# huangjh-pub/di-fusion

Hardware: AMD Instinct MI355X
Metric: frames/s integrate+decode+mesh, 640x480 synthetic stream (higher is better)
Workload: dtype f32

## Files before the change

### di_fusion_amd/csrc/common.hip.h

```cpp
#pragma once
#include <hip/hip_runtime.h>
#include <stdint.h>

#include "../../include/difusion.h"

#define DIF_WAVE 64
#define DIF_BLOCK 256
#define DIF_INVALID_KEY 0xFFFFFFFFu
#define NO_PACKED_F32 _Pragma("clang loop vectorize(disable) interleave(disable)")

#define DIF_CHECK_LAUNCH()                                   \
    do {                                                     \
        if (hipGetLastError() != hipSuccess) return DIF_ELAUNCH; \
    } while (0)

namespace dif {

struct Geo {
    int nx, ny, nz;
    float bx, by, bz, vs;
};

__host__ inline Geo geo_of(const dif_map_t* m) {
    Geo g;
    g.nx = m->nx; g.ny = m->ny; g.nz = m->nz;
    g.bx = m->bound_min[0]; g.by = m->bound_min[1]; g.bz = m->bound_min[2];
    g.vs = m->voxel_size;
    return g;
}

__device__ __forceinline__ int xcd_run_item(int b, int n, int max_run) {
    if (b >= n) return b;
    for (int base = 0, rem = n; rem >= 16;) {
        int R = 1 << (28 - __clz(rem));
        if (R > max_run) R = max_run;
        if (b < base + 8 * R) { const int l = b - base; return base + (l & 7) * R + (l >> 3); }
        base += 8 * R; rem -= 8 * R;
    }
    return b;
}

__device__ __forceinline__ int lane_id() { return (int)(threadIdx.x & 63); }

__device__ __forceinline__ float normalize1(float p, float b, float vs) { return __fdiv_rn(__fsub_rn(p, b), vs); }

__device__ __forceinline__ bool voxel_of(const Geo& g, float x, float y, float z, float& xnx, float& xny, float& xnz,
                                         int& ix, int& iy, int& iz) {
    xnx = normalize1(x, g.bx, g.vs);
    xny = normalize1(y, g.by, g.vs);
    xnz = normalize1(z, g.bz, g.vs);
    float cx = ceilf(xnx), cy = ceilf(xny), cz = ceilf(xnz);
    bool ok = (cx >= 1.0f) && (cy >= 1.0f) && (cz >= 1.0f) && (cx <= (float)g.nx) && (cy <= (float)g.ny) && (cz <= (float)g.nz);
    ix = ok ? (int)cx - 1 : 0;
    iy = ok ? (int)cy - 1 : 0;
    iz = ok ? (int)cz - 1 : 0;
    return ok;
}

__device__ __forceinline__ int linearize(const Geo& g, int ix, int iy, int iz) { return iz + g.nz * iy + (g.nz * g.ny) * ix; }

__device__ __forceinline__ void unlinearize(const Geo& g, int lin, int& ix, int& iy, int& iz) {
    ix = lin / (g.ny * g.nz);
    iy = (lin / g.nz) % g.ny;
    iz = lin % g.nz;
}

__device__ __forceinline__ int clampi(int v, int lo, int hi) { return v < lo ? lo : (v > hi ? hi : v); }

struct GridMarks {
    uint32_t* bits; int* tot; int per_words;
    __device__ __forceinline__ void set(int v) const {
        const uint32_t b = 1u << (v & 31);
        const int w = v >> 5;
        const uint32_t old = atomicOr(bits + w, b);
        if (!(old & b)) atomicAdd(tot + w / per_words, 1);
    }
};

struct HaloLists {
    int32_t* list; int cap; int* counters;
    int64_t l_lo, l_hi, r_lo, r_hi;
    __device__ __forceinline__ void note(int slot, int64_t lin) const {
        if (!list) return;
        if (lin >= l_lo && lin < l_hi) { const int k = atomicAdd(counters + DIF_C_HALO_L, 1); if (k < cap) list[k] = slot; }
        if (lin >= r_lo && lin < r_hi) { const int k = atomicAdd(counters + DIF_C_HALO_R, 1); if (k < cap) list[cap + k] = slot; }
    }
};

__host__ inline bool map_is_tiled(const dif_map_t* m) { return m->own_x_hi > m->own_x_lo && (m->own_x_lo > 0 || m->own_x_hi < m->nx); }

__host__ inline HaloLists halo_lists_of(const dif_map_t* m) {
    HaloLists h = {};
    if (!m->halo_list || m->halo_list_cap <= 0 || !map_is_tiled(m) || m->halo <= 0) return h;
    const int64_t plane = (int64_t)m->ny * m->nz;
    h.list = m->halo_list; h.cap = m->halo_list_cap; h.counters = m->counters;
    if (m->own_x_lo > 0) { h.l_lo = m->own_x_lo * plane; h.l_hi = (int64_t)(m->own_x_lo + m->halo < m->own_x_hi ? m->own_x_lo + m->halo : m->own_x_hi) * plane; }
    if (m->own_x_hi < m->nx) { h.r_hi = m->own_x_hi * plane; h.r_lo = (int64_t)(m->own_x_hi - m->halo > m->own_x_lo ? m->own_x_hi - m->halo : m->own_x_lo) * plane; }
    return h;
}

template <int CTRL, int ROW_MASK>
__device__ __forceinline__ long long dpp_mov64(long long v) {
    const int lo = __builtin_amdgcn_update_dpp(0, (int)v, CTRL, ROW_MASK, 0xF, false);
    const int hi = __builtin_amdgcn_update_dpp(0, (int)(v >> 32), CTRL, ROW_MASK, 0xF, false);
    return ((long long)hi << 32) | (unsigned int)lo;
}

__device__ __forceinline__ long long seg_incl_scan32(long long v, int col, int my_head) {
    const int head_r = max(my_head, col & 16);
    long long u;
    u = dpp_mov64<0x111, 0xF>(v); if (col - 1 >= head_r) v += u;
    u = dpp_mov64<0x112, 0xF>(v); if (col - 2 >= head_r) v += u;
    u = dpp_mov64<0x114, 0xF>(v); if (col - 4 >= head_r) v += u;
    u = dpp_mov64<0x118, 0xF>(v); if (col - 8 >= head_r) v += u;
    u = dpp_mov64<0x142, 0xA>(v); if (col >= 16 && my_head < 16) v += u;
    return v;
}

__device__ __forceinline__ int wave_incl_scan(int v) {
    int lane = lane_id();
#pragma unroll
    for (int d = 1; d < 64; d <<= 1) {
        int o = __shfl_up(v, d);
        if (lane >= d) v += o;
    }
    return v;
}

__device__ __forceinline__ int block_excl_scan(int v, int* smem, int& total) {
    int lane = lane_id(), wid = threadIdx.x >> 6, nw = blockDim.x >> 6;
    int inc = wave_incl_scan(v);
    __syncthreads();
    if (lane == 63) smem[wid] = inc;
    __syncthreads();
    int base = 0, tot = 0;
    for (int w = 0; w < nw; ++w) {
        int s = smem[w];
        if (w < wid) base += s;
        tot += s;
    }
    total = tot;
    return base + inc - v;
}

__device__ __forceinline__ int block_sum(int v, int* smem) {
    int lane = lane_id(), wid = threadIdx.x >> 6, nw = blockDim.x >> 6;
#pragma unroll
    for (int d = 32; d >= 1; d >>= 1) v += __shfl_xor(v, d);
    __syncthreads();
    if (lane == 0) smem[wid] = v;
    __syncthreads();
    int tot = 0;
    for (int w = 0; w < nw; ++w) tot += smem[w];
    return tot;
}

__device__ __forceinline__ void scan_range(int n, int& lo, int& hi) {
    int per = (n + (int)gridDim.x - 1) / (int)gridDim.x;
    per = (per + DIF_BLOCK - 1) / DIF_BLOCK * DIF_BLOCK;
    long long l = (long long)blockIdx.x * per;
    lo = l < n ? (int)l : n;
    long long h = l + per;
    hi = h < n ? (int)h : n;
}

template <class F>
__global__ void __launch_bounds__(DIF_BLOCK) k_scan_pass1(F f, const int* n_ptr, int n_static, int* block_tot) {
    __shared__ int smem[8];
    int n = n_ptr ? *n_ptr : n_static;
    int lo, hi;
    scan_range(n, lo, hi);
    int c = 0;
    for (int i = lo + (int)threadIdx.x; i < hi; i += DIF_BLOCK) c += f.count(i);
    int tot = block_sum(c, smem);
    if (threadIdx.x == 0) block_tot[blockIdx.x] = tot;
}

template <class F>
__global__ void __launch_bounds__(DIF_BLOCK) k_scan_pass2(F f, const int* n_ptr, int n_static, const int* block_tot) {
    __shared__ int smem[8];
    int n = n_ptr ? *n_ptr : n_static;
    int lo, hi;
    scan_range(n, lo, hi);
    int before = 0, all = 0;
    for (int b = (int)threadIdx.x; b < (int)gridDim.x; b += DIF_BLOCK) {
        int t = block_tot[b];
        all += t;
        if (b < (int)blockIdx.x) before += t;
    }
    int offset = block_sum(before, smem);
    int total = block_sum(all, smem);
    for (int base = lo; base < hi; base += DIF_BLOCK) {
        int i = base + (int)threadIdx.x;
        int c = (i < hi) ? f.count(i) : 0;
        int chunk_total;
        int ex = block_excl_scan(c, smem, chunk_total);
        if (i < hi && c > 0) f.emit(i, offset + ex);
        offset += chunk_total;
    }
    if (blockIdx.x == 0 && threadIdx.x == 0) f.finish(total);
}

template <class F>
__global__ void __launch_bounds__(1024) k_scan_single(F f, const int* n_ptr, int n_static) {
    __shared__ int smem[16];
    const int n = n_ptr ? *n_ptr : n_static;
    const int per = (n + 1023) / 1024;
    const int lo = min(n, (int)threadIdx.x * per), hi = min(n, lo + per);
    int c = 0;
    for (int i = lo; i < hi; ++i) c += f.count(i);
    int total;
    int offset = block_excl_scan(c, smem, total);
    for (int i = lo; i < hi; ++i) {
        int ci = f.count(i);
        if (ci > 0) f.emit(i, offset);
        offset += ci;
    }
    if (threadIdx.x == 0) f.finish(total);
}

template <class A, int NS>
struct BatchN { A s[NS]; };
template <class A>
using Batch = BatchN<A, DIF_MAX_STREAMS>;

template <int NS, class T>
struct Ranges {
    T pre[NS + 1], cnt[NS];
    __device__ __forceinline__ T total() const { return pre[NS]; }
    __device__ __forceinline__ void locate(T x, int& sm, T& lt, T& n) const {
        sm = 0; lt = x; n = cnt[0];
#pragma unroll
        for (int j = 1; j < NS; ++j)
            if (x >= pre[j]) { sm = j; lt = x - pre[j]; n = cnt[j]; }
    }
};

template <class F>
struct ScanBatch { F f[DIF_MAX_STREAMS]; const int* tot[DIF_MAX_STREAMS]; };

template <class F>
__global__ void __launch_bounds__(DIF_BLOCK) k_scan_pass2_batch(ScanBatch<F> b, int n_static) {
    __shared__ int smem[8];
    const F& f = b.f[blockIdx.y];
    const int* __restrict__ block_tot = b.tot[blockIdx.y];
    const int n = n_static;
    int lo, hi;
    scan_range(n, lo, hi);
    int before = 0, all = 0;
    for (int k = (int)threadIdx.x; k < (int)gridDim.x; k += DIF_BLOCK) {
        int t = block_tot[k];
        all += t;
        if (k < (int)blockIdx.x) before += t;
    }
    int offset = block_sum(before, smem);
    int total = block_sum(all, smem);
    for (int base = lo; base < hi; base += DIF_BLOCK) {
        int i = base + (int)threadIdx.x;
        int c = (i < hi) ? f.count(i) : 0;
        int chunk_total;
        int ex = block_excl_scan(c, smem, chunk_total);
        if (i < hi && c > 0) f.emit(i, offset + ex);
        offset += chunk_total;
    }
    if (blockIdx.x == 0 && threadIdx.x == 0) f.finish(total);
}

template <class F>
__global__ void __launch_bounds__(1024) k_scan_single_batch(ScanBatch<F> b, int n_static) {
    __shared__ int smem[16];
// ... 106 lines not shown
```

### di_fusion_amd/csrc/kernels_integrate.hip.h

```cpp
#pragma once

__device__ __forceinline__ void voxel_count_point(const Geo& g, bool in_range, float x, float y, float z, int64_t i, int* __restrict__ pt_lin,
                                                  int* __restrict__ frame_count, int* __restrict__ counters, int px_lo, int px_hi) {
    const int lane = lane_id();
    if (i < 4) counters[DIF_C_ALLOC_NEW + i] = 0;
    int lin = -2;
    if (in_range) {
        float xn, yn, zn; int ix, iy, iz;
        bool ok = voxel_of(g, x, y, z, xn, yn, zn, ix, iy, iz);
        ok = ok && ix >= px_lo && ix < px_hi;
        lin = ok ? linearize(g, ix, iy, iz) : -1;
        pt_lin[i] = lin;
    }
    int prev = __shfl_up(lin, 1);
    bool head = (lane == 0) || (prev != lin);
    unsigned long long heads = __ballot(head);
    if (head && lin >= 0) {
        unsigned long long above = (lane == 63) ? 0ull : (heads >> (lane + 1));
        int run = above ? __ffsll((long long)above) : (64 - lane);
        atomicAdd(frame_count + lin, run);
    }
}

__global__ void __launch_bounds__(DIF_BLOCK) k_voxel_count(Geo g, const float* __restrict__ xyz, int64_t N, int* __restrict__ pt_lin,
                                                         int* __restrict__ frame_count, int* __restrict__ counters, int px_lo, int px_hi) {
    const int64_t i = (int64_t)blockIdx.x * blockDim.x + threadIdx.x;
    const bool in = i < N;
    voxel_count_point(g, in, in ? xyz[i * 3 + 0] : 0.f, in ? xyz[i * 3 + 1] : 0.f, in ? xyz[i * 3 + 2] : 0.f, i, pt_lin, frame_count, counters, px_lo, px_hi);
}

struct ImageGeo { int H, W; float fx, fy, cx, cy; };

struct PointSrc {
    const float* xyz; const float* normal;
    const dif_frame_t* frame; ImageGeo im;
};

__device__ __forceinline__ Pose pose_of(const dif_frame_t* __restrict__ frame) {
    Pose P;
#pragma unroll
    for (int k = 0; k < 9; ++k) P.r[k] = frame->pose[k];
#pragma unroll
    for (int k = 0; k < 3; ++k) P.t[k] = frame->pose[9 + k];
    return P;
}

__device__ __forceinline__ void src_point(const PointSrc& s, const Pose& P, int64_t i, float (&p)[3]) {
    if (s.xyz) { p[0] = s.xyz[i * 3 + 0]; p[1] = s.xyz[i * 3 + 1]; p[2] = s.xyz[i * 3 + 2]; return; }
    float nv[3];
    unproject_point(s.frame->depth, nullptr, i, s.im.W, s.im.fx, s.im.fy, s.im.cx, s.im.cy, P, p, nv);
}

__device__ __forceinline__ void src_point_normal(const PointSrc& s, const Pose& P, int64_t i, float (&p)[3], float (&nv)[3]) {
    if (s.xyz) {
        p[0] = s.xyz[i * 3 + 0]; p[1] = s.xyz[i * 3 + 1]; p[2] = s.xyz[i * 3 + 2];
        nv[0] = s.normal[i * 3 + 0]; nv[1] = s.normal[i * 3 + 1]; nv[2] = s.normal[i * 3 + 2];
        return;
    }
    unproject_point(s.frame->depth, s.frame->normal_cam, i, s.im.W, s.im.fx, s.im.fy, s.im.cx, s.im.cy, P, p, nv);
}

__device__ __forceinline__ void unproject_voxel_count_body(const Geo& g, const dif_frame_t* __restrict__ frame, int H, int W, float fx, float fy,
                                                           float cx, float cy, float* __restrict__ xyz, float* __restrict__ nrm,
                                                           int* __restrict__ pt_lin, int* __restrict__ frame_count, int* __restrict__ counters,
                                                           int px_lo, int px_hi, const dif_pending_export_t* __restrict__ pending, int nb_x,
                                                           dif_frame_t* __restrict__ frame_copy, uint8_t* __restrict__ chunk_any) {
    if ((int)blockIdx.x < nb_x) {
        export_pending_rows(pending, (int)blockIdx.x, 3 * nb_x);
        return;
    }
    const int64_t N = (int64_t)H * W;
    const int64_t i = (int64_t)((int)blockIdx.x - nb_x) * blockDim.x + threadIdx.x;
    const bool in = i < N;
    if ((int)blockIdx.x == nb_x && threadIdx.x < 16 && frame_copy)
        reinterpret_cast<uint32_t*>(frame_copy)[threadIdx.x] = reinterpret_cast<const uint32_t*>(frame)[threadIdx.x];
    float p[3] = {0.f, 0.f, 0.f}, nv[3];
    if (in) {
        const Pose P = pose_of(frame);
        if (xyz) {
            unproject_point(frame->depth, frame->normal_cam, i, W, fx, fy, cx, cy, P, p, nv);
            xyz[i * 3 + 0] = p[0]; xyz[i * 3 + 1] = p[1]; xyz[i * 3 + 2] = p[2];
            nrm[i * 3 + 0] = nv[0]; nrm[i * 3 + 1] = nv[1]; nrm[i * 3 + 2] = nv[2];
        } else {
            unproject_point(frame->depth, nullptr, i, W, fx, fy, cx, cy, P, p, nv);
        }
    }
    voxel_count_point(g, in, p[0], p[1], p[2], i, pt_lin, frame_count, counters, px_lo, px_hi);
    if (chunk_any) {
        const int any = __syncthreads_or((int)(in && pt_lin[i] >= 0));
        if (threadIdx.x == 0) chunk_any[(int)blockIdx.x - nb_x] = (uint8_t)(any != 0);
    }
}

struct UvcArgs {
    Geo g; const dif_frame_t* frame; float* xyz; float* nrm; int* pt_lin; int* frame_count; int* counters; int px_lo, px_hi;
    const dif_pending_export_t* pending;
    dif_frame_t* frame_copy;
    uint8_t* chunk_any;
};

__global__ void __launch_bounds__(DIF_BLOCK) k_unproject_voxel_count(UvcArgs a, ImageGeo im, int nb_x) {
    unproject_voxel_count_body(a.g, a.frame, im.H, im.W, im.fx, im.fy, im.cx, im.cy, a.xyz, a.nrm, a.pt_lin, a.frame_count, a.counters, a.px_lo, a.px_hi,
                               a.pending, nb_x, a.frame_copy, a.chunk_any);
}
__global__ void __launch_bounds__(DIF_BLOCK) k_unproject_voxel_count_batch(Batch<UvcArgs> b, ImageGeo im, int nb_x) {
    const UvcArgs& a = b.s[blockIdx.y];
    unproject_voxel_count_body(a.g, a.frame, im.H, im.W, im.fx, im.fy, im.cx, im.cy, a.xyz, a.nrm, a.pt_lin, a.frame_count, a.counters, a.px_lo, a.px_hi,
                               a.pending, nb_x, a.frame_copy, a.chunk_any);
}

__device__ __forceinline__ void prune_mark_body(const Geo& g, int prune_min, const int* __restrict__ pt_lin, int64_t N,
                                                const int* __restrict__ frame_count, const int64_t* __restrict__ indexer,
                                                uint8_t* __restrict__ unq_mask, const GridMarks& marks,
                                                int* __restrict__ counters, const dif_pending_export_t* __restrict__ pending, int nb_x,
                                                const uint8_t* __restrict__ chunk_any) {
    if ((int)blockIdx.x < nb_x) {
        export_pending_rows(pending, nb_x + (int)blockIdx.x, 3 * nb_x);
        return;
    }
    const uint32_t* bits = marks.bits;
    int64_t i = (int64_t)((int)blockIdx.x - nb_x) * blockDim.x + threadIdx.x;
    if (chunk_any && !chunk_any[(int)blockIdx.x - nb_x]) {
        if (i < N) unq_mask[i] = 0;
        return;
    }
    int lane = lane_id();
    int lin = (i < N) ? pt_lin[i] : -2;
    bool keep = false;
    const int cnt = (lin >= 0) ? frame_count[lin] : 0;
    const int64_t own = (lin >= 0) ? indexer[lin] : 0;
    if (lin >= 0) keep = (prune_min > 0) ? (cnt > prune_min) : true;
    if (i < N) unq_mask[i] = keep ? 1 : 0;
    int prev = __shfl_up(lin, 1);
    bool head = (lane == 0) || (prev != lin);
    if (head && keep && own == -1) {
        int ix, iy, iz;
        unlinearize(g, lin, ix, iy, iz);
        int cand[7];
        cand[0] = lin;
        cand[1] = linearize(g, clampi(ix - 1, 0, g.nx - 1), iy, iz);
        cand[2] = linearize(g, clampi(ix + 1, 0, g.nx - 1), iy, iz);
        cand[3] = linearize(g, ix, clampi(iy - 1, 0, g.ny - 1), iz);
        cand[4] = linearize(g, ix, clampi(iy + 1, 0, g.ny - 1), iz);
        cand[5] = linearize(g, ix, iy, clampi(iz - 1, 0, g.nz - 1));
        cand[6] = linearize(g, ix, iy, clampi(iz + 1, 0, g.nz - 1));
        bool empty[7];
#pragma unroll
        for (int c = 0; c < 7; ++c) empty[c] = indexer[cand[c]] == -1;
        uint32_t prev[7];
#pragma unroll
        for (int c = 0; c < 7; ++c) {
            const uint32_t b = 1u << (cand[c] & 31);
            prev[c] = (!empty[c] || (bits[cand[c] >> 5] & b)) ? 0xFFFFFFFFu : atomicOr(marks.bits + (cand[c] >> 5), b);
        }
#pragma unroll
        for (int c = 0; c < 7; ++c)
            if (!(prev[c] & (1u << (cand[c] & 31)))) atomicAdd(marks.tot + (cand[c] >> 5) / marks.per_words, 1);
    }
}

struct PruneArgs {
    Geo g; int prune_min; const int* pt_lin; const int* frame_count; const int64_t* indexer; uint8_t* unq_mask; GridMarks marks; int* counters;
    const dif_pending_export_t* pending; const uint8_t* chunk_any;
};

__global__ void __launch_bounds__(DIF_BLOCK) k_prune_mark(PruneArgs a, int64_t N, int nb_x) {
    prune_mark_body(a.g, a.prune_min, a.pt_lin, N, a.frame_count, a.indexer, a.unq_mask, a.marks, a.counters, a.pending, nb_x, a.chunk_any);
}
__global__ void __launch_bounds__(DIF_BLOCK) k_prune_mark_batch(Batch<PruneArgs> b, int64_t N, int nb_x) {
    const PruneArgs& a = b.s[blockIdx.y];
    prune_mark_body(a.g, a.prune_min, a.pt_lin, N, a.frame_count, a.indexer, a.unq_mask, a.marks, a.counters, a.pending, nb_x, a.chunk_any);
}

struct AllocFunctor {
    uint32_t* bits;
    int64_t* indexer;
    int64_t* pos;
    int* counters;
    int64_t capacity;
    HaloLists hl;
    __device__ int count(int w) const { return __popc(bits[w]); }
    __device__ void emit(int w, int offset) const {
        uint32_t word = bits[w];
        bits[w] = 0u;
        int base = counters[DIF_C_N_OCCUPIED] + offset;
        while (word) {
            int b = __ffs((int)word) - 1;
            word &= word - 1;
            int lin = w * 32 + b;
            if (base < capacity) {
                indexer[lin] = base;
                pos[base] = lin;
                hl.note(base, lin);
            }
            ++base;
        }
    }
    __device__ void finish(int total) const { counters[DIF_C_ALLOC_NEW] = total; }
};

__device__ __forceinline__ bool in_encode_set(int64_t slot, const float* __restrict__ obs, float th) { return slot >= 0 && obs[slot] < th; }

#define FG_TABLE 256
__device__ __forceinline__ void focus_gather_body(const Geo& g, float enc_th, const PointSrc& src, const int* __restrict__ pt_lin,
                                                  const uint8_t* __restrict__ unq_mask, int64_t N, int* __restrict__ frame_count,
                                                  const int64_t* __restrict__ indexer, const float* __restrict__ obs,
                                                  uint2* __restrict__ pair_list, int* __restrict__ counters, int64_t capacity, int img_w,
                                                  int* __restrict__ grid_tot, int own_lo, int own_hi,
                                                  const dif_pending_export_t* __restrict__ pending, int nb_x, const uint8_t* __restrict__ chunk_any) {
    if ((int)blockIdx.x < nb_x) {
        export_pending_rows(pending, 2 * nb_x + (int)blockIdx.x, 3 * nb_x);
        return;
// ... 16 lines not shown
    }
    if (i == 0) {
        int n = counters[DIF_C_N_OCCUPIED] + counters[DIF_C_ALLOC_NEW];
        if (n > capacity) { n = (int)capacity; counters[DIF_C_OVERFLOW] = 1; }
        counters[DIF_C_N_OCCUPIED] = n;
    }
    if (chunk_any && img_w > 0) {
        int flag = 0;
        if (threadIdx.x < 16) flag = chunk_any[(i + (int64_t)threadIdx.x * img_w) >> 8];
        if (!__syncthreads_or(flag)) return;
    }
    const int lin = (i < N) ? pt_lin[i] : -1;
    uint32_t key[8];
#pragma unroll
    for (int o = 0; o < 8; ++o) key[o] = DIF_INVALID_KEY;
    const int lane = lane_id(), wid = (int)(threadIdx.x >> 6);
    const bool kept = lin >= 0 && unq_mask[i];
    if (lin >= 0) frame_count[lin] = 0;
    const int prev = __shfl_up(lin, 1);
    const bool head = (lane == 0) || (prev != lin);
    const unsigned long long heads = __ballot(head);
    bool focus = false;
    if (head && kept) {
        int ix, iy, iz;
        unlinearize(g, lin, ix, iy, iz);
        const int plane = g.ny * g.nz;
        const int nl[7] = {lin, lin - plane, lin + plane, lin - g.nz, lin + g.nz, lin - 1, lin + 1};
        const bool in_grid[7] = {true, ix > 0, ix < g.nx - 1, iy > 0, iy < g.ny - 1, iz > 0, iz < g.nz - 1};
        int64_t slot[7];
#pragma unroll
        for (int q = 0; q < 7; ++q) slot[q] = in_grid[q] ? indexer[nl[q]] : -1;
        float w[7];
#pragma unroll
        for (int q = 0; q < 7; ++q) w[q] = slot[q] >= 0 ? obs[slot[q]] : enc_th;
#pragma unroll
        for (int q = 0; q < 7; ++q) focus |= w[q] < enc_th;
    }
    const int my_head = 63 - __clzll((long long)(heads & ((2ull << lane) - 1ull)));
    focus = __shfl((int)focus, my_head) != 0;
    if (kept && focus) {
        float xn, yn, zn; int ix, iy, iz;
        float p[3];
        src_point(src, src.xyz ? Pose{} : pose_of(src.frame), i, p);
        voxel_of(g, p[0], p[1], p[2], xn, yn, zn, ix, iy, iz);
        int64_t slot[8];
#pragma unroll
        for (int o = 0; o < 8; ++o) {
            float ox = (o & 4) ? 0.5f : -0.5f, oy = (o & 2) ? 0.5f : -0.5f, oz = (o & 1) ? 0.5f : -0.5f;
            int gx = clampi((int)(ceilf(xn + ox) - 1.0f), 0, g.nx - 1);
            int gy = clampi((int)(ceilf(yn + oy) - 1.0f), 0, g.ny - 1);
            int gz = clampi((int)(ceilf(zn + oz) - 1.0f), 0, g.nz - 1);
            slot[o] = (gx >= own_lo && gx < own_hi) ? indexer[linearize(g, gx, gy, gz)] : -1;
        }
        float w[8];
#pragma unroll
        for (int o = 0; o < 8; ++o) w[o] = slot[o] >= 0 ? obs[slot[o]] : enc_th;
#pragma unroll
        for (int o = 0; o < 8; ++o)
            if (w[o] < enc_th) key[o] = (uint32_t)slot[o];
    }
    bool any = false;
#pragma unroll
    for (int o = 0; o < 8; ++o) any |= key[o] != DIF_INVALID_KEY;
    if (!__syncthreads_or((int)any)) return;
    int where[8], rank[8];
#pragma unroll
    for (int o = 0; o < 8; ++o) {
        where[o] = -1; rank[o] = 0;
        if (key[o] == DIF_INVALID_KEY) continue;
        unsigned h = (key[o] * 2654435761u) >> 24;
        for (int probes = 0; probes < FG_TABLE; ++probes) {
            const unsigned old = atomicCAS(tkey + h, DIF_INVALID_KEY, key[o]);
            if (old == DIF_INVALID_KEY || old == key[o]) { where[o] = (int)h; break; }
            h = (h + 1) & (FG_TABLE - 1);
        }
        rank[o] = atomicAdd(where[o] >= 0 ? tcnt + where[o] : &s_loose, 1);
    }
    __syncthreads();
    int grouped;
    const int first = block_excl_scan(tcnt[threadIdx.x], smem, grouped);
    __syncthreads();
    tcnt[threadIdx.x] = first;
    if (threadIdx.x == 0) s_base = atomicAdd(counters + DIF_C_M, grouped + s_loose);
    __syncthreads();
#pragma unroll
    for (int o = 0; o < 8; ++o)
        if (key[o] != DIF_INVALID_KEY)
            pair_list[s_base + (where[o] >= 0 ? tcnt[where[o]] : grouped) + rank[o]] = make_uint2(key[o], (uint32_t)((int64_t)o * N + i));
}

struct GatherArgs {
    Geo g; float enc_th; PointSrc src; const int* pt_lin; const uint8_t* unq_mask; int* frame_count; const int64_t* indexer; const float* obs;
    uint2* pair_list; int* counters; int64_t capacity; int* grid_tot; int own_lo, own_hi; const dif_pending_export_t* pending; const uint8_t* chunk_any;
};

__global__ void __launch_bounds__(DIF_BLOCK) k_focus_gather(GatherArgs a, int64_t N, int img_w, int nb_x) {
    focus_gather_body(a.g, a.enc_th, a.src, a.pt_lin, a.unq_mask, N, a.frame_count, a.indexer, a.obs, a.pair_list, a.counters, a.capacity, img_w, a.grid_tot,
                      a.own_lo, a.own_hi, a.pending, nb_x, a.chunk_any);
}
__global__ void __launch_bounds__(DIF_BLOCK) k_focus_gather_batch(Batch<GatherArgs> b, int64_t N, int img_w, int nb_x) {
    const GatherArgs& a = b.s[blockIdx.y];
    focus_gather_body(a.g, a.enc_th, a.src, a.pt_lin, a.unq_mask, N, a.frame_count, a.indexer, a.obs, a.pair_list, a.counters, a.capacity, img_w, a.grid_tot,
                      a.own_lo, a.own_hi, a.pending, nb_x, a.chunk_any);
}

#define DIF_FIX_SCALE 1073741824.0f
#define DIF_REC_WORDS 32
#define DIF_REC_COUNT_POS 29
#define DIF_DIR_WORDS 16
#define DIF_DIR_IDS (DIF_DIR_WORDS - 2)
#define DIF_REC_POISON_SHIFT 40

#ifdef DIF_TRACE
__device__ unsigned long long g_en_trace[4096 * 8];
#define EN_STAMP(slot) do { if (lane_id() == 0) g_en_trace[((threadIdx.x >> 6) * gridDim.x + blockIdx.x) * 8 + (slot)] = wall_clock64(); } while (0)
#else
#define EN_STAMP(slot) do { } while (0)
#endif

struct EncArgs {
    Geo g; PointSrc src; const uint2* pair_list; int* rec_dir; int* rec_next; long long* rec; int* upd_list; int* counters;
    uint8_t* dirty; int* dirty_tot;
};
#ifndef ENC_X6_THREADS
#define ENC_X6_THREADS 768
#endif
template <bool X6, int NS>
__device__ __forceinline__ void encode_body(const BatchN<EncArgs, NS>& B, int S, const float* __restrict__ wblob, int64_t N) {
    extern __shared__ __attribute__((aligned(16))) float lds[];
    EN_STAMP(0);
    const int lane = lane_id(), half = lane >> 5, col = lane & 31;
    const int wave = __builtin_amdgcn_readfirstlane((int)((threadIdx.x >> 6) * gridDim.x + blockIdx.x));
    const int nwaves = (int)(gridDim.x * (blockDim.x >> 6));
    Ranges<NS, int> rg;
    rg.pre[0] = 0;
#pragma unroll
    for (int j = 0; j < NS; ++j) {
        rg.cnt[j] = (j < S) ? B.s[j].counters[DIF_C_M] : 0;
        rg.pre[j + 1] = rg.pre[j] + ((rg.cnt[j] + 31) >> 5);
    }
    const int n_tiles = rg.total();
    struct TileIn { uint2 e; float x0, x1, x2; };
    auto gather = [&](bool any, int sm, int lt, int M) __attribute__((always_inline)) {
        TileIn t;
        t.e = make_uint2(DIF_INVALID_KEY, 0u);
        t.x0 = t.x1 = t.x2 = 0.f;
        if (any) {
            const EncArgs& a = B.s[sm];
            const Geo g = a.g;
            const int row = lt * 32 + col;
            if (row < M) {
                t.e = a.pair_list[row];
                const uint32_t v = t.e.y;
                int o = 0;
#pragma unroll
                for (int k = 1; k < 8; ++k) o += ((int64_t)v >= (int64_t)k * N) ? 1 : 0;
                int64_t i = (int64_t)v - (int64_t)o * N;
                float pw[3], nw[3];
                src_point_normal(a.src, a.src.xyz ? Pose{} : pose_of(a.src.frame), i, pw, nw);
                float xn = normalize1(pw[0], g.bx, g.vs);
                float yn = normalize1(pw[1], g.by, g.vs);
                float zn = normalize1(pw[2], g.bz, g.vs);
                float ox = (o & 4) ? 0.5f : -0.5f, oy = (o & 2) ? 0.5f : -0.5f, oz = (o & 1) ? 0.5f : -0.5f;
                float gx = (float)clampi((int)(ceilf(xn + ox) - 1.0f), 0, g.nx - 1);
                float gy = (float)clampi((int)(ceilf(yn + oy) - 1.0f), 0, g.ny - 1);
                float gz = (float)clampi((int)(ceilf(zn + oz) - 1.0f), 0, g.nz - 1);
                float rx = (xn - gx) - 0.5f, ry = (yn - gy) - 0.5f, rz = (zn - gz) - 0.5f;
                float nxv = nw[0], nyv = nw[1], nzv = nw[2];
                t.x0 = half ? ry : rx;
                t.x1 = half ? nxv : rz;
                t.x2 = half ? nzv : nyv;
            }
        }
        return t;
    };
    int sm_n, lt_n, M_n;
    rg.locate(wave, sm_n, lt_n, M_n);
    TileIn nxt = gather(wave < n_tiles, sm_n, lt_n, M_n);
    __builtin_amdgcn_sched_barrier(0);
    stage_weights(lds, wblob, X6 ? E6_BYTES / 4 : ENC_FLOATS);
    EN_STAMP(1);
    for (int T = wave; T < n_tiles; T += nwaves) {
        const TileIn cur = nxt;
        const int sm = sm_n, tile = lt_n, M = M_n;
        rg.locate(T + nwaves, sm_n, lt_n, M_n);
        nxt = gather(T + nwaves < n_tiles, sm_n, lt_n, M_n);
        const EncArgs& a = B.s[sm];
        const int row = tile * 32 + col;
        const bool live = row < M;
        const uint2 e = cur.e;
        const uint32_t key = e.x;
        const uint32_t key_prev = (uint32_t)__shfl_up((int)key, 1), key_next = (uint32_t)__shfl_down((int)key, 1);
        const bool run_head = (col == 0) || (key_prev != key);
        const bool run_tail = (col == 31) || (key_next != key);
        const uint32_t heads32 = (uint32_t)(__ballot(run_head) >> (half * 32));
        const int my_head = 31 - __clz((int)(heads32 & ((2u << col) - 1u)));
        const int rec_id = tile * 32 + __popc(heads32 & ((2u << col) - 1u)) - 1;
        const float x0 = cur.x0, x1 = cur.x1, x2 = cur.x2;
        unsigned nf = (((__float_as_uint(x0) & 0x7f800000u) == 0x7f800000u) || ((__float_as_uint(x1) & 0x7f800000u) == 0x7f800000u) ||
                       ((__float_as_uint(x2) & 0x7f800000u) == 0x7f800000u)) ? 1u : 0u;
        nf |= (unsigned)__shfl_xor((int)nf, 32);
        EN_STAMP(2);
        int dir_pos = 0;
        const bool pusher = live && run_tail && half == 0;
        int* dir = a.rec_dir + (int64_t)key * DIF_DIR_WORDS;
        if (pusher) dir_pos = atomicAdd(dir, 1);
        f16v out;
        if constexpr (X6) out = encoder_tile_x6(lds, x0, x1, x2, lane);
        else out = encoder_tile(lds, x0, x1, x2, lane);
        EN_STAMP(3);
        long long* p = a.rec + (int64_t)rec_id * DIF_REC_WORDS + half * 16;
#pragma unroll
        for (int r = 0; r < 16; ++r) {
            long long v = live ? __float2ll_rn(out[r] * DIF_FIX_SCALE) : 0ll;
            if (half == 1 && r == 13) v = live ? 1ll + ((long long)nf << DIF_REC_POISON_SHIFT) : 0ll;
            v = seg_incl_scan32(v, col, my_head);
            if (live && run_tail) p[r] = v;
        }
        if (pusher) {
            if (dir_pos < DIF_DIR_IDS) dir[2 + dir_pos] = rec_id;
            else a.rec_next[rec_id] = atomicExch(dir + 1, rec_id + 1);
            if (dir_pos == 0) {
                a.upd_list[atomicAdd(a.counters + DIF_C_C, 1)] = (int)key;
                if (a.dirty_tot && !a.dirty[key]) atomicAdd(a.dirty_tot + (key >> 8), 1);
            }
        }
        EN_STAMP(4);
    }
    EN_STAMP(5);
}

template <bool X6>
__global__ void __launch_bounds__(X6 ? ENC_X6_THREADS : 512, X6 ? 1 : 2)
k_encode(Geo g, const float* __restrict__ wblob, const float* __restrict__ xyz, const float* __restrict__ normal, const dif_frame_t* __restrict__ frame,
         ImageGeo im, int64_t N, const uint2* __restrict__ pair_list, int* __restrict__ rec_dir, int* __restrict__ rec_next, long long* __restrict__ rec,
         int* __restrict__ upd_list, int* __restrict__ counters, uint8_t* __restrict__ dirty, int* __restrict__ dirty_tot) {
    const BatchN<EncArgs, 1> B{{EncArgs{g, PointSrc{xyz, normal, frame, im}, pair_list, rec_dir, rec_next, rec, upd_list, counters, dirty, dirty_tot}}};
    encode_body<X6, 1>(B, 1, wblob, N);
}

template <bool X6>
__global__ void __launch_bounds__(X6 ? ENC_X6_THREADS : 512, X6 ? 1 : 2)
k_encode_batch(Batch<EncArgs> B, int S, const float* __restrict__ wblob, int64_t N) {
    encode_body<X6, DIF_MAX_STREAMS>(B, S, wblob, N);
}

template <bool X6>
__global__ void __launch_bounds__(512, X6 ? 1 : 2) k_encode_rows(const float* __restrict__ wblob, const float* __restrict__ rows, int64_t n, float* __restrict__ out) {
    extern __shared__ __attribute__((aligned(16))) float lds[];
    stage_weights(lds, wblob, X6 ? E6_BYTES / 4 : ENC_FLOATS);
    const int lane = lane_id(), half = lane >> 5, col = lane & 31;
    const int wave = (int)((threadIdx.x >> 6) * gridDim.x + blockIdx.x);
    const int nwaves = (int)(gridDim.x * (blockDim.x >> 6));
    const int64_t n_tiles = (n + 31) / 32;
    for (int64_t tile = wave; tile < n_tiles; tile += nwaves) {
        int64_t row = tile * 32 + col;
        bool live = row < n;
        float x0 = 0.f, x1 = 0.f, x2 = 0.f;
        if (live) {
            const float* p = rows + row * 6;
            x0 = half ? p[1] : p[0];
            x1 = half ? p[3] : p[2];
            x2 = half ? p[5] : p[4];
        }
        unsigned nf = (((__float_as_uint(x0) & 0x7f800000u) == 0x7f800000u) || ((__float_as_uint(x1) & 0x7f800000u) == 0x7f800000u) ||
                       ((__float_as_uint(x2) & 0x7f800000u) == 0x7f800000u)) ? 1u : 0u;
        nf |= (unsigned)__shfl_xor((int)nf, 32);
        f16v o;
        if constexpr (X6) o = encoder_tile_x6(lds, x0, x1, x2, lane);
        else o = encoder_tile(lds, x0, x1, x2, lane);
        if (live) {
#pragma unroll
            for (int r = 0; r < 16; ++r) {
                int f = (r & 3) + 8 * (r >> 2) + 4 * half;
                if (f < L) out[row * L + f] = nf ? __builtin_nanf("") : o[r];
            }
        }
    }
}

__device__ __forceinline__ void fuse_body(const long long* __restrict__ rec, const int* __restrict__ rec_next, int* __restrict__ rec_dir,
                                          const int* __restrict__ upd_list, float* __restrict__ latent, float* __restrict__ obs,
                                          uint8_t* __restrict__ dirty, int* __restrict__ counters, const int64_t* __restrict__ slot_lin, const HaloLists& hl,
                                          dif_pending_export_t* __restrict__ pending, int* __restrict__ dirty_tot, int* __restrict__ fc) {
    if (pending && blockIdx.x == 0 && threadIdx.x == 0) {
        pending->pending = 0;
        if (pending->notify) {
            __threadfence_system();
            *pending->notify = pending->seq;
        }
    }
    const int n_upd = counters[DIF_C_C];
    const int first_new = counters[DIF_C_N_OCCUPIED] - counters[DIF_C_ALLOC_NEW];
    const int grp = (int)((blockIdx.x * blockDim.x + threadIdx.x) >> 5), ngrp = (int)((gridDim.x * blockDim.x) >> 5);
    const int f = threadIdx.x & 31;
    const int pos = ((f >> 2) & 1) * 16 + (f & 3) + 4 * (f >> 3);
    for (int u = grp; u < n_upd; u += ngrp) {
        const int s = upd_list[u];
        int* dir = rec_dir + (int64_t)s * DIF_DIR_WORDS;
        const int n_rec = dir[0];
        const int my_id = (f < DIF_DIR_IDS && f < n_rec) ? dir[2 + f] : -1;
        const float w_old = obs[s];
        const float z_old = f < L ? latent[(int64_t)s * L + f] : 0.0f;
        long long Si = 0;
        long long len = 0;
        const int n_dir = n_rec < DIF_DIR_IDS ? n_rec : DIF_DIR_IDS;
        for (int j = 0; j < n_dir; ++j) {
            const long long* r = rec + (int64_t)__shfl(my_id, j, 32) * DIF_REC_WORDS;
            Si += r[pos];
            len += r[DIF_REC_COUNT_POS];
        }
        if (n_rec > DIF_DIR_IDS)
            for (int id = dir[1]; id != 0; id = rec_next[id - 1]) {
                const long long* r = rec + (int64_t)(id - 1) * DIF_REC_WORDS;
                Si += r[pos];
                len += r[DIF_REC_COUNT_POS];
            }
        const int cnt = (int)(len & ((1ll << DIF_REC_POISON_SHIFT) - 1));
        if (f < L) {
            float S = (float)Si * (1.0f / DIF_FIX_SCALE);
            S = S + z_old * w_old;
            float w_new = w_old + (float)cnt;
            latent[(int64_t)s * L + f] = (len >> DIF_REC_POISON_SHIFT) ? __builtin_nanf("") : S / w_new;
        }
        if (my_id >= 0) dir[2 + f] = 0;
        __builtin_amdgcn_wave_barrier();
        if (f == 31) {
            obs[s] = w_old + (float)cnt;
            if (dirty_tot && !dirty[s]) atomicAdd(dirty_tot + (s >> 8), 1);
            dirty[s] = 1;
            dir[0] = 0;
            dir[1] = 0;
            if (hl.list && s < first_new) hl.note(s, slot_lin[s]);
        }
    }
    if (blockIdx.x == 0 && threadIdx.x == 0) {
        const int items = (counters[DIF_C_M] + 31) >> 5;
        counters[DIF_C_ITEMS] = items;
        if (fc) {
            fc[DIF_FC_SHADOW + 0] = counters[DIF_C_N_OCCUPIED]; fc[DIF_FC_SHADOW + 1] = counters[DIF_C_ALLOC_NEW];
            fc[DIF_FC_SHADOW + 2] = counters[DIF_C_M]; fc[DIF_FC_SHADOW + 3] = counters[DIF_C_C]; fc[DIF_FC_SHADOW + 4] = items;
        }
    }
}

struct FuseArgs {
    const long long* rec; const int* rec_next; int* rec_dir; const int* upd_list; float* latent; float* obs; uint8_t* dirty; int* counters;
    const int64_t* slot_lin; HaloLists hl; dif_pending_export_t* pending;
    int* dirty_tot; int* fc;
};

__global__ void __launch_bounds__(DIF_BLOCK) k_fuse(FuseArgs a) {
    fuse_body(a.rec, a.rec_next, a.rec_dir, a.upd_list, a.latent, a.obs, a.dirty, a.counters, a.slot_lin, a.hl, a.pending, a.dirty_tot, a.fc);
}
__global__ void __launch_bounds__(DIF_BLOCK) k_fuse_batch(Batch<FuseArgs> b) {
    const FuseArgs& a = b.s[blockIdx.y];
    fuse_body(a.rec, a.rec_next, a.rec_dir, a.upd_list, a.latent, a.obs, a.dirty, a.counters, a.slot_lin, a.hl, a.pending, a.dirty_tot, a.fc);
}
```

### di_fusion_amd/csrc/kernels_points.hip.h

```cpp
#pragma once

__global__ void __launch_bounds__(DIF_BLOCK) k_unproject(const float* __restrict__ depth, float* __restrict__ pc, int H, int W,
                                                       float fx, float fy, float cx, float cy) {
    int64_t n = (int64_t)H * W;
    for (int64_t i = (int64_t)blockIdx.x * blockDim.x + threadIdx.x; i < n; i += (int64_t)gridDim.x * blockDim.x) {
        int v = (int)(i / W), u = (int)(i - (int64_t)v * W);
        float d = depth[i];
        float x, y, z;
        if (d == d) {
            x = ((float)u - cx) / fx * d;
            y = ((float)v - cy) / fy * d;
            z = d;
        } else {
            x = y = z = __builtin_nanf("");
        }
        pc[i * 3 + 0] = x; pc[i * 3 + 1] = y; pc[i * 3 + 2] = z;
    }
}

struct Pose { float r[9]; float t[3]; };

__device__ __forceinline__ void unproject_point(const float* __restrict__ depth, const float* __restrict__ ncam, int64_t i, int W, float fx, float fy,
                                                float cx, float cy, const Pose& P, float (&p)[3], float (&nv)[3]) {
    const int v = (int)(i / W), u = (int)(i - (int64_t)v * W);
    const float d = depth[i];
    const float qnan = __builtin_nanf("");
    p[0] = p[1] = p[2] = nv[0] = nv[1] = nv[2] = qnan;
    if (d == d) {
        const float x = ((float)u - cx) / fx * d;
        const float y = ((float)v - cy) / fy * d;
        const float z = d;
        p[0] = ((P.r[0] * x + P.r[1] * y) + P.r[2] * z) + P.t[0];
        p[1] = ((P.r[3] * x + P.r[4] * y) + P.r[5] * z) + P.t[1];
        p[2] = ((P.r[6] * x + P.r[7] * y) + P.r[8] * z) + P.t[2];
        if (ncam) {
            const float a = ncam[i * 3 + 0], b = ncam[i * 3 + 1], c = ncam[i * 3 + 2];
            nv[0] = (P.r[0] * a + P.r[1] * b) + P.r[2] * c;
            nv[1] = (P.r[3] * a + P.r[4] * b) + P.r[5] * c;
            nv[2] = (P.r[6] * a + P.r[7] * b) + P.r[8] * c;
        }
    }
}

__device__ __forceinline__ void copy_dwords_strided(const uint32_t* __restrict__ src, uint32_t* __restrict__ dst, int64_t n, int64_t t0, int64_t stride) {
    int64_t j = t0;
    for (; j + 3 * stride < n; j += 4 * stride) {
        const uint32_t a = src[j], b = src[j + stride], c = src[j + 2 * stride], d = src[j + 3 * stride];
        dst[j] = a; dst[j + stride] = b; dst[j + 2 * stride] = c; dst[j + 3 * stride] = d;
    }
    for (; j < n; j += stride) dst[j] = src[j];
}

__device__ __forceinline__ void export_pending_rows(const dif_pending_export_t* __restrict__ d, int part, int nparts) {
    if (!d->pending) return;
    const int64_t kept = d->kept, n = d->n;
    const int64_t stride = (int64_t)nparts * blockDim.x, t0 = (int64_t)part * blockDim.x + threadIdx.x;
    copy_dwords_strided(reinterpret_cast<const uint32_t*>(d->log_tri + kept * 9), reinterpret_cast<uint32_t*>(d->out_tri), n * 9, t0, stride);
    copy_dwords_strided(reinterpret_cast<const uint32_t*>(d->log_std + kept * 3), reinterpret_cast<uint32_t*>(d->out_std), n * 3, t0, stride);
    copy_dwords_strided(reinterpret_cast<const uint32_t*>(d->log_id + kept), reinterpret_cast<uint32_t*>(d->out_id), n * 2, t0, stride);
}

#define DIF_EXPORT_WGS 64

__global__ void __launch_bounds__(DIF_BLOCK) k_export_pending(dif_pending_export_t* __restrict__ d) {
    export_pending_rows(d, (int)blockIdx.x, (int)gridDim.x);
}

__global__ void __launch_bounds__(DIF_BLOCK) k_unproject_transform(const float* __restrict__ depth, const float* __restrict__ ncam,
                                                                 float* __restrict__ xyz, float* __restrict__ nrm, int H, int W,
                                                                 float fx, float fy, float cx, float cy, Pose P, const float* __restrict__ pose_dev,
                                                                 const dif_frame_t* __restrict__ frame) {
    if (frame) {
        depth = frame->depth;
        ncam = frame->normal_cam;
        pose_dev = frame->pose;
    }
    if (pose_dev) {
#pragma unroll
        for (int i = 0; i < 9; ++i) P.r[i] = pose_dev[i];
#pragma unroll
        for (int i = 0; i < 3; ++i) P.t[i] = pose_dev[9 + i];
    }
    int64_t n = (int64_t)H * W;
    for (int64_t i = (int64_t)blockIdx.x * blockDim.x + threadIdx.x; i < n; i += (int64_t)gridDim.x * blockDim.x) {
        float p[3], nv[3];
        unproject_point(depth, ncam, i, W, fx, fy, cx, cy, P, p, nv);
        xyz[i * 3 + 0] = p[0]; xyz[i * 3 + 1] = p[1]; xyz[i * 3 + 2] = p[2];
        if (nrm) { nrm[i * 3 + 0] = nv[0]; nrm[i * 3 + 1] = nv[1]; nrm[i * 3 + 2] = nv[2]; }
    }
}

struct V3 { float x, y, z; };

__device__ __forceinline__ V3 backproject(int u, int v, float d, float fx, float fy, float cx, float cy) {
    const float qnan = __builtin_nanf("");
    if (!(d == d)) return V3{qnan, qnan, qnan};
    return V3{((float)u - cx) / fx * d, ((float)v - cy) / fy * d, d};
}

__device__ __forceinline__ bool normal_weight_of(const V3& c, const V3& xp, const V3& xm, const V3& yp, const V3& ym, float (&o)[4]) {
    if (c.z <= 1e-6) return false;
    if (xp.z < 1e-6 || xm.z < 1e-6 || yp.z < 1e-6 || ym.z < 1e-6) return false;
    const float dxx = xp.x - xm.x, dxy = xp.y - xm.y, dxz = xp.z - xm.z;
    const float dyx = yp.x - ym.x, dyy = yp.y - ym.y, dyz = yp.z - ym.z;
    float nx = dyy * dxz - dyz * dxy, ny = dyz * dxx - dyx * dxz, nz = dyx * dxy - dyy * dxx;
    const float len = sqrtf(nx * nx + ny * ny + nz * nz);
    if (len < 1e-6) return false;
    nx /= len; ny /= len; nz /= len;
    const float theta = acosf(nz);
    const float td = theta / (0.5f * 3.14159f - theta);
    const float wgt = (0.0012f + 0.0019f * (c.z - 0.4f) * (c.z - 0.4f) + 0.0001f / sqrtf(c.z) * td * td);
    o[0] = nx; o[1] = ny; o[2] = nz; o[3] = 1.0f / wgt;
    return true;
}

#define FE_TILE 16
#define FE_RAW (FE_TILE + 6)
#define FE_FIL (FE_TILE + 2)

struct FrontendArgs {
    const float* depth; int H, W;
    float fx, fy, cx, cy;
    int filter;
    float* depth_out; int write_border;
    float* pc;
    float* normal_weight;
    float* frame_depth;
    float* frame_normal;
};

__global__ void __launch_bounds__(FE_TILE * FE_TILE) k_depth_frontend(FrontendArgs a) {
    __shared__ float raw[FE_RAW][FE_RAW + 1];
    __shared__ float fil[FE_FIL][FE_FIL + 1];
    const int u0 = (int)blockIdx.x * FE_TILE, v0 = (int)blockIdx.y * FE_TILE, t = (int)threadIdx.x;
    const float qnan = __builtin_nanf("");
    for (int k = t; k < FE_RAW * FE_RAW; k += FE_TILE * FE_TILE) {
        const int i = k / FE_RAW, j = k % FE_RAW, v = v0 - 3 + i, u = u0 - 3 + j;
        raw[i][j] = (v >= 0 && v < a.H && u >= 0 && u < a.W) ? a.depth[(int64_t)v * a.W + u] : qnan;
    }
    __syncthreads();
    const float sig_l2 = 1.2232f * 1.2232f;
    for (int k = t; k < FE_FIL * FE_FIL; k += FE_TILE * FE_TILE) {
        const int i = k / FE_FIL, j = k % FE_FIL, v = v0 - 1 + i, u = u0 - 1 + j;
        float z = raw[i + 2][j + 2];
        if (a.filter && v >= 2 && v < a.H - 2 && u >= 2 && u < a.W - 2) {
            if (z < 1e-6) {
                z = 0.0f;
            } else {
                const float sigma_z = 1.0f / (0.0012f + 0.0019f * (z - 0.4f) * (z - 0.4f) + 0.0001f / sqrtf(z) * 0.25f);
                float w_sum = 0.0f, acc = 0.0f;
                for (int di = -2; di <= 2; ++di)
                    for (int dj = -2; dj <= 2; ++dj) {
                        const float nz = raw[i + 2 + di][j + 2 + dj];
                        if (nz < 1e-6) continue;
                        const float dz = (nz - z) * (nz - z);
                        const float wgt = expf(-0.5f * ((float)(abs(di) + abs(dj)) * sig_l2 + dz * sigma_z * sigma_z));
                        w_sum += wgt;
                        acc += wgt * nz;
                    }
                z = acc / w_sum;
            }
        }
        fil[i][j] = z;
    }
    __syncthreads();
    const int lx = t & (FE_TILE - 1), ly = t / FE_TILE, u = u0 + lx, v = v0 + ly;
    if (u >= a.W || v >= a.H) return;
    const int64_t px = (int64_t)v * a.W + u;
    const float d = fil[ly + 1][lx + 1];
    const bool interior = v >= 2 && v < a.H - 2 && u >= 2 && u < a.W - 2;
    if (a.depth_out && (interior || a.write_border)) a.depth_out[px] = d;
    const V3 c = backproject(u, v, d, a.fx, a.fy, a.cx, a.cy);
    if (a.pc) { a.pc[px * 3 + 0] = c.x; a.pc[px * 3 + 1] = c.y; a.pc[px * 3 + 2] = c.z; }
    if (!a.normal_weight && !a.frame_normal) return;
    float o[4] = {0.0f, 0.0f, 0.0f, -1.0f};
    bool ok = false;
    if (!(v < 1 || v > a.H - 2 || u < 1 || u > a.W - 2))
        ok = normal_weight_of(c, backproject(u + 1, v, fil[ly + 1][lx + 2], a.fx, a.fy, a.cx, a.cy),
                              backproject(u - 1, v, fil[ly + 1][lx], a.fx, a.fy, a.cx, a.cy),
                              backproject(u, v + 1, fil[ly + 2][lx + 1], a.fx, a.fy, a.cx, a.cy),
                              backproject(u, v - 1, fil[ly][lx + 1], a.fx, a.fy, a.cx, a.cy), o);
    if (a.normal_weight) {
        if (ok) { a.normal_weight[px * 4 + 0] = o[0]; a.normal_weight[px * 4 + 1] = o[1]; a.normal_weight[px * 4 + 2] = o[2]; }
        a.normal_weight[px * 4 + 3] = ok ? o[3] : -1.0f;
    }
    if (a.frame_normal) {
        const bool use = ok && o[3] > 0.0f && (o[0] == o[0]) && (d == d);
        a.frame_depth[px] = use ? d : qnan;
        a.frame_normal[px * 3 + 0] = use ? o[0] : qnan; a.frame_normal[px * 3 + 1] = use ? o[1] : qnan; a.frame_normal[px * 3 + 2] = use ? o[2] : qnan;
    }
}

__global__ void __launch_bounds__(FE_TILE * FE_TILE) k_normal_weight(const float* __restrict__ pc, float* __restrict__ out, int H, int W) {
    __shared__ float tile[FE_FIL][FE_FIL][3];
    const int u0 = (int)blockIdx.x * FE_TILE, v0 = (int)blockIdx.y * FE_TILE, t = (int)threadIdx.x;
// ... 137 lines not shown
```

Measured before the change: 10010.

## Split fixed-point scan into 32-bit halves and cheapen encoder gather index math

```diff
diff --git a/di_fusion_amd/csrc/common.hip.h b/di_fusion_amd/csrc/common.hip.h
--- a/di_fusion_amd/csrc/common.hip.h
+++ b/di_fusion_amd/csrc/common.hip.h
@@ -106,16 +106,49 @@
     return ((long long)hi << 32) | (unsigned int)lo;
 }
 
-__device__ __forceinline__ long long seg_incl_scan32(long long v, int col, int my_head) {
-    const int head_r = max(my_head, col & 16);
+struct SegSteps {
+    bool s1, s2, s4, s8, sx;
+    __device__ __forceinline__ SegSteps(int col, int my_head) {
+        const int head_r = max(my_head, col & 16);
+        s1 = col - 1 >= head_r; s2 = col - 2 >= head_r; s4 = col - 4 >= head_r; s8 = col - 8 >= head_r;
+        sx = col >= 16 && my_head < 16;
+    }
+};
+__device__ __forceinline__ long long seg_incl_scan32(long long v, const SegSteps& st) {
     long long u;
-    u = dpp_mov64<0x111, 0xF>(v); if (col - 1 >= head_r) v += u;
-    u = dpp_mov64<0x112, 0xF>(v); if (col - 2 >= head_r) v += u;
-    u = dpp_mov64<0x114, 0xF>(v); if (col - 4 >= head_r) v += u;
-    u = dpp_mov64<0x118, 0xF>(v); if (col - 8 >= head_r) v += u;
-    u = dpp_mov64<0x142, 0xA>(v); if (col >= 16 && my_head < 16) v += u;
+    u = dpp_mov64<0x111, 0xF>(v); if (st.s1) v += u;
+    u = dpp_mov64<0x112, 0xF>(v); if (st.s2) v += u;
+    u = dpp_mov64<0x114, 0xF>(v); if (st.s4) v += u;
+    u = dpp_mov64<0x118, 0xF>(v); if (st.s8) v += u;
+    u = dpp_mov64<0x142, 0xA>(v); if (st.sx) v += u;
     return v;
 }
+__device__ __forceinline__ long long seg_incl_scan32(long long v, int col, int my_head) { return seg_incl_scan32(v, SegSteps(col, my_head)); }
+
+#define DIF_FIX_SPLIT_BITS 21
+#define DIF_FIX_SPLIT_MAX_BITS 0x57000000u
+struct Fix2 { int h, l; };
+__device__ __forceinline__ Fix2 fix_split(float v) {
+    const float H = truncf(v * (1.0f / (float)(1 << DIF_FIX_SPLIT_BITS)));
+    const float l = fmaf(H, -(float)(1 << DIF_FIX_SPLIT_BITS), v);
+    return Fix2{(int)H, (int)rintf(l)};
+}
+__device__ __forceinline__ long long fix_join(int h, int l) { return (long long)h * (1 << DIF_FIX_SPLIT_BITS) + (long long)l; }
+
+template <int CTRL, int ROW_MASK>
+__device__ __forceinline__ int dpp_add(int v) { return v + __builtin_amdgcn_update_dpp(0, v, CTRL, ROW_MASK, 0xF, false); }
+__device__ __forceinline__ int incl_scan32(int v) {
+    v = dpp_add<0x111, 0xF>(v);
+    v = dpp_add<0x112, 0xF>(v);
+    v = dpp_add<0x114, 0xF>(v);
+    v = dpp_add<0x118, 0xF>(v);
+    return dpp_add<0x142, 0xA>(v);
+}
+struct RunPrev {
+    int addr, mask;
+    __device__ __forceinline__ RunPrev(int half, int my_head) : addr((half * 32 + max(my_head - 1, 0)) << 2), mask(my_head > 0 ? -1 : 0) {}
+    __device__ __forceinline__ int of(int prefix) const { return __builtin_amdgcn_ds_bpermute(addr, prefix) & mask; }
+};
 
 __device__ __forceinline__ int wave_incl_scan(int v) {
     int lane = lane_id();
diff --git a/di_fusion_amd/csrc/kernels_integrate.hip.h b/di_fusion_amd/csrc/kernels_integrate.hip.h
--- a/di_fusion_amd/csrc/kernels_integrate.hip.h
+++ b/di_fusion_amd/csrc/kernels_integrate.hip.h
@@ -58,6 +58,18 @@
         return;
     }
     unproject_point(s.frame->depth, s.frame->normal_cam, i, s.im.W, s.im.fx, s.im.fy, s.im.cx, s.im.cy, P, p, nv);
+}
+
+__device__ __forceinline__ void src_point_normal_u32(const PointSrc& s, const Pose& P, uint32_t i, float (&p)[3], float (&nv)[3]) {
+    if (s.xyz) {
+        const int64_t j = (int64_t)i * 3;
+        p[0] = s.xyz[j + 0]; p[1] = s.xyz[j + 1]; p[2] = s.xyz[j + 2];
+        nv[0] = s.normal[j + 0]; nv[1] = s.normal[j + 1]; nv[2] = s.normal[j + 2];
+        return;
+    }
+    int u, v;
+    PixDiv(s.im.W).split(i, u, v);
+    unproject_pixel<true>(s.frame->depth, s.frame->normal_cam, i, u, v, s.im.fx, s.im.fy, s.im.cx, s.im.cy, P, p, nv);
 }
 
 __device__ __forceinline__ void unproject_voxel_count_body(const Geo& g, const dif_frame_t* __restrict__ frame, int H, int W, float fx, float fy,
@@ -380,12 +392,13 @@
             if (row < M) {
                 t.e = a.pair_list[row];
                 const uint32_t v = t.e.y;
+                const uint32_t Nu = (uint32_t)N;
                 int o = 0;
 #pragma unroll
-                for (int k = 1; k < 8; ++k) o += ((int64_t)v >= (int64_t)k * N) ? 1 : 0;
-                int64_t i = (int64_t)v - (int64_t)o * N;
+                for (int k = 1; k < 8; ++k) o += (v >= (uint32_t)k * Nu) ? 1 : 0;
+                const uint32_t i = v - (uint32_t)o * Nu;
                 float pw[3], nw[3];
-                src_point_normal(a.src, a.src.xyz ? Pose{} : pose_of(a.src.frame), i, pw, nw);
+                src_point_normal_u32(a.src, a.src.xyz ? Pose{} : pose_of(a.src.frame), i, pw, nw);
                 float xn = normalize1(pw[0], g.bx, g.vs);
                 float yn = normalize1(pw[1], g.by, g.vs);
                 float zn = normalize1(pw[2], g.bz, g.vs);
@@ -438,12 +451,41 @@
         else out = encoder_tile(lds, x0, x1, x2, lane);
         EN_STAMP(3);
         long long* p = a.rec + (int64_t)rec_id * DIF_REC_WORDS + half * 16;
+        float v[16];
+        unsigned vmax = 0u;
 #pragma unroll
         for (int r = 0; r < 16; ++r) {
-            long long v = live ? __float2ll_rn(out[r] * DIF_FIX_SCALE) : 0ll;
-            if (half == 1 && r == 13) v = live ? 1ll + ((long long)nf << DIF_REC_POISON_SHIFT) : 0ll;
-            v = seg_incl_scan32(v, col, my_head);
-            if (live && run_tail) p[r] = v;
+            v[r] = out[r] * DIF_FIX_SCALE;
+            vmax = max(vmax, __float_as_uint(v[r]) & 0x7fffffffu);
+        }
+        if (__builtin_expect(__ballot(live && vmax >= DIF_FIX_SPLIT_MAX_BITS) != 0ull, 0)) {
+            int col_here = col;
+            asm volatile("" : "+v"(col_here));
+            const SegSteps steps(col_here, my_head);
+#pragma unroll
+            for (int r = 0; r < 16; ++r) {
+                long long s = live ? __float2ll_rn(v[r]) : 0ll;
+                if (half == 1 && r == 13) s = live ? 1ll + ((long long)nf << DIF_REC_POISON_SHIFT) : 0ll;
+                s = seg_incl_scan32(s, steps);
+                if (live && run_tail) p[r] = s;
+            }
+        } else {
+            const RunPrev prev(half, my_head);
+            long long s[16];
+#pragma unroll
+            for (int r = 0; r < 16; ++r) {
+                Fix2 q = fix_split(live ? v[r] : 0.f);
+                if (half == 1 && r == 13) {
+                    q.h = live ? (int)(nf << (DIF_REC_POISON_SHIFT - DIF_FIX_SPLIT_BITS)) : 0;
+                    q.l = live ? 1 : 0;
+                }
+                const int ph = incl_scan32(q.h), pl = incl_scan32(q.l);
+                s[r] = fix_join(ph - prev.of(ph), pl - prev.of(pl));
+            }
+            if (live && run_tail) {
+#pragma unroll
+                for (int r = 0; r < 16; ++r) p[r] = s[r];
+            }
         }
         if (pusher) {
             if (dir_pos < DIF_DIR_IDS) dir[2 + dir_pos] = rec_id;
diff --git a/di_fusion_amd/csrc/kernels_points.hip.h b/di_fusion_amd/csrc/kernels_points.hip.h
--- a/di_fusion_amd/csrc/kernels_points.hip.h
+++ b/di_fusion_amd/csrc/kernels_points.hip.h
@@ -20,10 +20,12 @@
 
 struct Pose { float r[9]; float t[3]; };
 
-__device__ __forceinline__ void unproject_point(const float* __restrict__ depth, const float* __restrict__ ncam, int64_t i, int W, float fx, float fy,
+template <bool EAGER_N = false, typename I = int64_t>
+__device__ __forceinline__ void unproject_pixel(const float* __restrict__ depth, const float* __restrict__ ncam, I i, int u, int v, float fx, float fy,
                                                 float cx, float cy, const Pose& P, float (&p)[3], float (&nv)[3]) {
-    const int v = (int)(i / W), u = (int)(i - (int64_t)v * W);
     const float d = depth[i];
+    float a = 0.f, b = 0.f, c = 0.f;
+    if (EAGER_N && ncam) { a = ncam[(int64_t)i * 3 + 0]; b = ncam[(int64_t)i * 3 + 1]; c = ncam[(int64_t)i * 3 + 2]; }
     const float qnan = __builtin_nanf("");
     p[0] = p[1] = p[2] = nv[0] = nv[1] = nv[2] = qnan;
     if (d == d) {
@@ -34,13 +36,29 @@
         p[1] = ((P.r[3] * x + P.r[4] * y) + P.r[5] * z) + P.t[1];
         p[2] = ((P.r[6] * x + P.r[7] * y) + P.r[8] * z) + P.t[2];
         if (ncam) {
-            const float a = ncam[i * 3 + 0], b = ncam[i * 3 + 1], c = ncam[i * 3 + 2];
+            if (!EAGER_N) { a = ncam[(int64_t)i * 3 + 0]; b = ncam[(int64_t)i * 3 + 1]; c = ncam[(int64_t)i * 3 + 2]; }
             nv[0] = (P.r[0] * a + P.r[1] * b) + P.r[2] * c;
             nv[1] = (P.r[3] * a + P.r[4] * b) + P.r[5] * c;
             nv[2] = (P.r[6] * a + P.r[7] * b) + P.r[8] * c;
         }
     }
 }
+
+__device__ __forceinline__ void unproject_point(const float* __restrict__ depth, const float* __restrict__ ncam, int64_t i, int W, float fx, float fy,
+                                                float cx, float cy, const Pose& P, float (&p)[3], float (&nv)[3]) {
+    const int v = (int)(i / W), u = (int)(i - (int64_t)v * W);
+    unproject_pixel(depth, ncam, i, u, v, fx, fy, cx, cy, P, p, nv);
+}
+
+struct PixDiv {
+    uint32_t W, m;
+    __device__ __forceinline__ explicit PixDiv(int w) : W((uint32_t)w), m((uint32_t)__builtin_amdgcn_readfirstlane((int)(0xFFFFFFFFu / (uint32_t)w))) {}
+    __device__ __forceinline__ void split(uint32_t i, int& u, int& v) const {
+        uint32_t q = __umulhi(i, m), r = i - q * W;
+        if (r >= W) { ++q; r -= W; }
+        u = (int)r; v = (int)q;
+    }
+};
 
 __device__ __forceinline__ void copy_dwords_strided(const uint32_t* __restrict__ src, uint32_t* __restrict__ dst, int64_t n, int64_t t0, int64_t stride) {
     int64_t j = t0;
```

Measured after the change: 9273. 7.4% lower.
